# tgcsaba/GPSig

Measured on AMD Instinct MI355X. Metric: sequence-pairs/sec for SignatureKernel.K (N,L,d,sig_level); fp64 rel-err vs ref, higher is better.
Workload: dtype f64; 1 GPU; BASELINE.json configs[1]: full N x N Gram, SignatureLinear, N=4096, L=64, d=8, num_levels=5, order=1, normalization=on, fp64, white-noise inputs

## Files before the change

### gpsig_amd/csrc/api.hip

```cpp
#include <hip/hip_runtime.h>

#include <cstdarg>
#include <cstdio>
#include <cstdlib>
#include <cstring>
#include <string>
#include <vector>

#include "../../include/gpsig_hip.h"
#include "aux_kernels.hpp"
#include "lowrank_kernels.hpp"
#include "lr_fused_args.hpp"
#include "lr_draw_kernels.hpp"
#include "seq_args.hpp"
#include "seq_configs.hpp"
#include "tvs_tile_kernel.hpp"
#include "seq_pk2_kernel.hpp"
#include "sig_feat_kernel.hpp"

namespace gpsig {
typedef hipError_t (*TvsTileLaunchFn)(TvsTileArgs&, size_t, hipStream_t, int);
TvsTileLaunchFn tvs_tile_lookup(int M, int NW, int D, bool incr, int kind);
TvsTileLaunchFn tvs_tile_lookup_ho(int M, int NW, int D, bool incr);
int tvs_tile_width(int d);
// ... 633 lines not shown
    if (x_squared && (X2 == nullptr || raw || !p->normalization)) return GPSIG_OK;
    if (f32 && (row_end > 0 || row_block_call)) return GPSIG_OK;
    if (c->shard_n > 1) return GPSIG_OK;
    const int M = p->num_levels;
    if (M < 2 || p->order < 1 || p->order > M) return GPSIG_OK;
    const int d = p->num_features * ((raw ? 0 : p->num_lags) + 1);
    SigFeatLaunchFn ffn = sig_feat_lookup(d, M);
    if (!ffn) return GPSIG_OK;
    const bool sym = X2 == nullptr;
    void* out32 = nullptr;
    const void* const X_given = X;
    const int64_t F = sig_feature_count(d, M), ld = (F + 1 + 15) / 16 * 16;
    const int r1 = p->difference ? L1 - 1 : L1, r2 = p->difference ? L2 - 1 : L2;
    if (r1 < 1 || r2 < 1) return GPSIG_OK;
    if (c->sig_features < 0 && d != 1) {
        const double lattice = double(r1) * r2 * (2.0 * d + 3.0 * M - 1.0) * (p->order > 1 ? 8.0 : 1.0) * (cosine ? 1.5 : 1.0) * (f32 ? 0.5 : 1.0), feat = 2.0 * double(F);
        const double pairs = sym ? double(N1) * N1 / 2 : double(N1) * N2;
        if (!(feat * 0.6 < lattice)) return GPSIG_OK;
        const double seqs = double(N1) + (sym ? 0.0 : double(N2)), t_seq = 60e-6 * double(sig_ipow(d, M)) / 32768.0;
        const double t_feat_kernel = ceil(seqs / 256.0) * t_seq > 15e-6 ? ceil(seqs / 256.0) * t_seq : 15e-6;
        const double t_lattice = 100e-6 + pairs * lattice / (d > 8 ? 12.5e12 : 25e12), t_features = 60e-6 + t_feat_kernel + pairs * feat / 60e12;
        if (pairs < 1024.0 || !(t_features < t_lattice)) return GPSIG_OK;
    }
    const size_t lds = sig_features_lds_bytes(d, M, L1 > L2 ? L1 : L2);
    if (lds > 150 * 1024) return GPSIG_OK;
    const bool rows = row_end > 0 || row_block_call;
    const int64_t NA = rows ? row_end - row_begin : N1, H = N1 / 2;
    int64_t NB = sym ? N1 : N2;
    if (rows) NB = (NA + H < N1) ? NA + H : N1;
    const int nti = int((NA + SG_BM - 1) / SG_BM), ntj = int((NB + SG_BN - 1) / SG_BN);
    const bool symtiles = sym && !rows;
    const int ntiles = symtiles ? nti * (nti + 1) / 2 : nti * ntj;
    const int nslab_all = int((ld + SG_BK - 1) / SG_BK);
    int nsplit = 1, graded = 1;
    {
        const int64_t nt_full = (N1 + SG_BM - 1) / SG_BM;
        const int64_t tiles_full = sym ? nt_full * (nt_full + 1) / 2 : nt_full * ((N2 + SG_BN - 1) / SG_BN);
        const double result_bytes = 8.0 * double(N1) * double(sym ? N1 : N2) * (sym ? 0.5 : 1.0);
        double best = 1e300;
        for (int ns = 1; ns <= 128 && ns * 8 <= nslab_all + 7; ++ns) {
            const double wgs = double(tiles_full) * ns, per_piece = double(nslab_all) / ns;
            const double t = (wgs <= 256.0 ? per_piece * 1.8e-6 + 10e-6 : ceil(wgs / 512.0) * (per_piece * 3.6e-6 + 10e-6)) +
                             (ns > 1 ? 2.0 * ns * result_bytes / 3e12 : 0.0);
            if (t < best * 0.999) { best = t; nsplit = ns; }
        }
        if (tiles_full > 1024 && nsplit < 4 && nslab_all >= 32) nsplit = 4;
        const double wgs = double(tiles_full) * nsplit, piece_t = double(nslab_all) / nsplit * 3.6e-6;
        if (c->sig_graded != 0 && wgs > 512.0 && nslab_all / nsplit >= 32) {
            const double rounds = wgs / 512.0, waste_equal = (ceil(rounds) - rounds) * piece_t;
            double best_t = waste_equal;
            for (int g = 2; g <= 5; ++g) {
                const double t = piece_t / double(1 << (g - 1)) + (g - 1) * 2.0 * result_bytes / 3e12;
                if (t < best_t * 0.95 && (nslab_all / nsplit) >> (g - 1) >= 8) { best_t = t; graded = g; }
            }
        }
    }
    const size_t part_one = sizeof(double) * size_t(NA) * NB;
    while (nsplit > 1 && part_one * size_t(nsplit - 1 + graded) > (size_t(40) << 30)) { --nsplit; graded = 1; }
    const int npieces = nsplit - 1 + graded;
    const size_t feat_bytes = sizeof(double) * size_t(ld) * (size_t(N1) + (sym ? 0 : size_t(N2)));
    if (feat_bytes + part_one * size_t(npieces) > (size_t(96) << 30)) return GPSIG_OK;
    {
        auto grow = [&](int id, size_t bytes) { return bytes > c->buf[id].cap ? bytes + bytes / 8 + 256 : size_t(0); };
        const size_t extra = grow(B_SF0, sizeof(double) * size_t(ld) * N1 + 64) + (sym ? 0 : grow(B_SF1, sizeof(double) * size_t(ld) * N2 + 64)) +
                             grow(B_SF2, part_one * size_t(npieces) + 64);
        if (extra > (size_t(1) << 30) && !c->capturing && !rows) {
            size_t free_b = 0, total_b = 0;
            if (hipMemGetInfo(&free_b, &total_b) == hipSuccess) {
                size_t held = 0;
                for (int id : {int(B_SF0), int(B_SF1), int(B_SF2)}) held += grow(id, id == B_SF0 ? sizeof(double) * size_t(ld) * N1 + 64 : id == B_SF1 ? (sym ? 0 : sizeof(double) * size_t(ld) * N2 + 64) : part_one * size_t(npieces) + 64) ? c->buf[id].cap : 0;
                if (extra > free_b + held - (free_b + held) / 16) return GPSIG_OK;
            }
        }
    }
    if (rows && NA <= 0) { *done = true; return GPSIG_OK; }
    const double* w = nullptr;
    if (!raw) CHK(upload_weights(c, p, &w));
    ScaleParams s;
    CHK(scale_params(c, p, !raw, &s));
    void *phi1, *phi2 = nullptr, *part;
    CHK(ensure(c, B_SF0, sizeof(double) * size_t(ld) * N1 + 64, &phi1));
    if (!sym) CHK(ensure(c, B_SF1, sizeof(double) * size_t(ld) * N2 + 64, &phi2));
    CHK(ensure(c, B_SF2, part_one * size_t(npieces) + 64, &part));
    if (f32) {
        void *x64, *y64 = nullptr, *o64;
        const int64_t per1 = int64_t(L1) * p->num_features, per2 = int64_t(L2) * p->num_features;
        CHK(ensure(c, B_SF3, sizeof(double) * size_t(N1 * per1) + 64, &x64));
        HIPCHK(c, sig_convert_launch(X, x64, N1 * per1, true, c->stream));
        if (!sym) {
            CHK(ensure(c, B_SF4, sizeof(double) * size_t(N2 * per2) + 64, &y64));
            HIPCHK(c, sig_convert_launch(X2, y64, N2 * per2, true, c->stream));
        }
        CHK(ensure(c, B_SF5, sizeof(double) * size_t(return_levels ? M + 1 : 1) * size_t(N1) * size_t(sym ? N1 : N2) + 64, &o64));
        out32 = out; X = x64; X2 = sym ? nullptr : y64; out = o64;
    }
    const int normalize = (!raw && p->normalization) ? 1 : 0;
    auto features = [&](const void* Xs, int64_t N, int L, void* phi, bool squared) -> int {
        SigFeatArgs A;
        memset(&A, 0, sizeof(A));
        A.X = static_cast<const double*>(Xs); A.N = N; A.L = L; A.difference = p->difference ? 1 : 0; A.P = s;
        A.w = w; A.normalize = normalize; A.jitter = p->jitter; A.Phi = static_cast<double*>(phi); A.ld = ld; A.dlev = nullptr;
        A.order = p->order;
        A.unit_points = cosine ? 1 : 0;
        A.norm_squared = squared ? 1 : 0;
        const int64_t cap = sig_threads(d, M) <= 128 ? 16384 : 4096;
        const unsigned grid = unsigned(N < cap ? N : cap);
        hipError_t e = ffn(A, grid, sig_features_lds_bytes(d, M, L), c->stream);
        if (e != hipSuccess) return fail(c, GPSIG_ERR_HIP, "sig_features_kernel: %s", hipGetErrorString(e));
        return GPSIG_OK;
    };
    uint64_t key = 1469598103934665603ull;
    auto mix = [&](const void* ptr, size_t bytes) {
        const unsigned char* b = static_cast<const unsigned char*>(ptr);
        for (size_t i = 0; i < bytes; ++i) { key ^= b[i]; key *= 1099511628211ull; }
    };
    {
        const int32_t head[8] = {p->base_kernel, p->dtype, p->num_features, p->num_levels, p->order, p->difference, p->normalization, p->num_lags};
        mix(head, sizeof(head));
        mix(&p->sigma, sizeof(double)); mix(&p->jitter, sizeof(double));
        mix(p->variances, sizeof(double) * (M + 1));
        if (p->lengthscales) mix(p->lengthscales, sizeof(double) * p->num_features);
        if (p->num_lags > 0) { mix(p->lags, sizeof(double) * p->num_lags); mix(p->gamma, sizeof(double) * (p->num_lags + 1)); }
        const int64_t tail[4] = {N1, L1, (raw ? 1 : 0) + (x_squared ? 2 : 0), ld};
        mix(tail, sizeof(tail));
    }
    const bool reuse = c->sf_keep && c->sf_valid && c->sf_X == X_given && c->sf_phi == phi1 && c->sf_key == key;
    if (N1 > 0 && !reuse) CHK(features(X, N1, L1, phi1, x_squared != 0));
    c->sf_valid = c->sf_keep != 0 && N1 > 0;
    c->sf_X = X_given; c->sf_phi = phi1; c->sf_key = key;
    if (!sym && N2 > 0) CHK(features(X2, N2, L2, phi2, false));
    if (NA <= 0 || NB <= 0) { *done = true; return GPSIG_OK; }
    const int nlev = return_levels ? M + 1 : 1;
    const int64_t Ncols = sym ? N1 : N2;
    for (int lv = 0; lv < nlev; ++lv) {
        int kb = 0, ke = int(F) + 1;
        double dval = 0.0;
        if (return_levels) {
            if (lv == 0) { kb = int(F); ke = int(F) + 1; }
            else { kb = sig_feature_count(d, lv - 1); ke = sig_feature_count(d, lv); }
            dval = raw ? 0.0 : p->sigma * p->variances[lv];
        } else {
            for (int m = 0; m <= M; ++m) dval += p->sigma * p->variances[m];
        }
        SigGramArgs G;
        memset(&G, 0, sizeof(G));
        G.A = static_cast<const double*>(phi1) + (rows ? row_begin * ld : 0);
        G.B = static_cast<const double*>(sym ? phi1 : phi2);
        G.NA = NA; G.NB = NB; G.lda = ld; G.ldb = ld;
        G.b_off = rows ? ((row_begin - H) % N1 + N1) % N1 : 0; G.b_mod = sym ? N1 : N2;
        G.k_begin = kb; G.k_end = ke;
        G.band = (rows && NA + H <= N1) ? H : 0;
        const int nslab = (ke - kb + SG_BK - 1) / SG_BK;
        const int ns = sig_piece_bounds(nslab, nsplit, return_levels ? 1 : graded, G.bound);
        G.nsplit = ns; G.symmetric = symtiles ? 1 : 0; G.ntj = ntj; G.part = static_cast<double*>(part);
        hipEvent_t e0 = nullptr, e1 = nullptr;
        bool on = false;
        if (timed) CHK(timing_begin_any(c, &e0, &e1, &on));
        int used_dma = 0;
        HIPCHK(c, sig_gram_launch(G, ntiles, c->stream, (c->sig_gemm_dma && !return_levels) ? 1 : 0, &used_dma));
        if (on) {
            HIPCHK(c, hipEventRecord(e1, c->stream));
            c->t_launches += 1;
            c->t_pairs += NA * NB;
            c->t_kernel = used_dma ? "sig_gram_dma_kernel" : "sig_gram_kernel";
            c->t_flops += 2.0 * double(ntiles) * SG_BM * SG_BN * double(nslab) * SG_BK;
        }
        SigReduceArgs R;
        memset(&R, 0, sizeof(R));
        R.part = static_cast<const double*>(part); R.nsplit = ns; R.NA = NA; R.NB = NB;
        R.out = static_cast<double*>(out) + (return_levels ? int64_t(lv) * N1 * Ncols : 0);
        R.so_i = Ncols; R.so_j = 1;
        R.mode = rows ? 2 : (symtiles ? 1 : 0);
        R.diag_set = (sym && normalize) ? 1 : 0; R.diag_value = dval;
        R.N = N1; R.r0 = row_begin; R.c0 = G.b_off; R.compact = compact;
        HIPCHK(c, sig_reduce_launch(R, c->stream));
    }
    if (out32) HIPCHK(c, sig_convert_launch(out, out32, int64_t(return_levels ? M + 1 : 1) * N1 * (sym ? N1 : N2), false, c->stream));
    *done = true;
    return GPSIG_OK;
}

template <typename TT>
struct Impl {
struct SeqPlanned {
    SeqConfig cfg;
    SeqLaunchFn fn;
    int mode, d_eff;
    bool rbf_prescaled;
    int fast_kind;
    double prescale;
    bool pk2;
    int ny, waves;
};

static int plan_seq(gpsig_ctx* c, const gpsig_params* p, int d_eff, int Ly, SeqPlanned* out, int64_t pairs_hint = 0) {
    SeqGeom g0 = seq_geometry(p->base_kernel, p->difference, Ly, 4, int(sizeof(TT)));
    out->rbf_prescaled = false;
    out->fast_kind = -1;
    out->prescale = 1.0;
    out->pk2 = false;
    out->ny = 1; out->waves = 1;
    if (p->base_kernel == GPSIG_BASE_SPECTRAL) {
        int k = -1;
        if (sizeof(TT) == 8 && c->spectral_wave != 0 && g0.mode == MODE_PT_DIFF && !(p->order > 1 && p->num_levels > 1))
            k = seq_select(SEQ_TABLE_SPECTRAL, N_SEQ_TABLE_SPECTRAL, g0.rows, d_eff, p->num_levels, false);
        if (k < 0) return fail(c, GPSIG_ERR_UNSUPPORTED, "the spectral base kernel: no wavefront kernel for this shape / dtype / order");
        out->cfg = SEQ_TABLE_SPECTRAL[k];
        out->mode = g0.mode;
        out->d_eff = d_eff;
        out->fn = out->cfg.G == 16 ? seq_lookup_ptd_spectral_g16(out->cfg.G, out->cfg.C, out->cfg.D, out->cfg.MMAX, false)
                                   : seq_lookup_ptd_spectral_g64(out->cfg.G, out->cfg.C, out->cfg.D, out->cfg.MMAX, false);
        if (!out->fn) return fail(c, GPSIG_ERR_UNSUPPORTED, "spectral seq-gram kernel shape missing from this build");
        return GPSIG_OK;
    }
    if (p->order > 1 && p->num_levels > 1) {
        int k = seq_select_ho(SEQ_HO_TABLE, N_SEQ_HO_TABLE, g0.rows, d_eff, p->num_levels, p->order);
        if (k < 0)
            return fail(c, GPSIG_ERR_UNSUPPORTED,
                        "no higher-order seq-gram kernel shape for %d record rows, d=%d, num_levels=%d, order=%d (built: order <= 8 up "
                        "to 64 rows, <= 4 up to 128 rows, 2 up to 512 rows; num_levels <= 6 (8 up to 64 rows); d <= 16, or d <= 32 with at most 128 rows)",
                        g0.rows, d_eff, p->num_levels, p->order);
        const SeqHOConfig& h = SEQ_HO_TABLE[k];
        out->cfg = SeqConfig{h.G, h.C, h.D, h.MMAX, false};
        out->mode = g0.mode;
        out->d_eff = d_eff;
        out->fn = seq_launcher_ho(g0.mode, h, sizeof(TT) == 4);
        if (sizeof(TT) == 8 && c->allow_exact && g0.mode == MODE_PT_DIFF && p->base_kernel == GPSIG_BASE_RBF) {
            SeqLaunchFn ex = seq_lookup_ho_ptdrbf_exact(h.G, h.C, h.D, p->num_levels, p->order);
            if (!ex) ex = seq_lookup_ho_ptdrbf_exact_o4(h.G, h.C, h.D, p->num_levels, p->order);
            if (ex) {
                out->fn = ex;
                out->cfg = SeqConfig{h.G, h.C, h.D, p->num_levels, true};
                out->rbf_prescaled = true;
                out->prescale = SEQ_RBF_PRESCALE;
            }
        }
        if (sizeof(TT) == 8 && c->allow_exact && g0.mode == MODE_PT_DIFF && seq_is_matern(p->base_kernel) && c->matern_fast != 0) {
            SeqLaunchFn ex = p->base_kernel == GPSIG_BASE_MATERN12 ? seq_lookup_ho_ptdm12_exact(BASE_MATERN12, h.G, h.C, h.D, p->num_levels, p->order)
                             : (p->base_kernel == GPSIG_BASE_MATERN32 ? seq_lookup_ho_ptdm32_exact(BASE_MATERN32, h.G, h.C, h.D, p->num_levels, p->order)
                                                                      : seq_lookup_ho_ptdm52_exact(BASE_MATERN52, h.G, h.C, h.D, p->num_levels, p->order));
            if (ex) {
                out->fn = ex;
                out->cfg = SeqConfig{h.G, h.C, h.D, p->num_levels, true};
                out->rbf_prescaled = true;
                out->prescale = seq_matern_prescale(p->base_kernel);
            }
        }
        if (!out->fn) return fail(c, GPSIG_ERR_UNSUPPORTED, "higher-order kernel shape missing from this build");
        return GPSIG_OK;
    }
    const bool f32 = sizeof(TT) == 4;
    if (f32 && c->allow_pk2 && c->allow_exact && (g0.mode == MODE_INC || (g0.mode == MODE_PT_DIFF && p->base_kernel == GPSIG_BASE_RBF))) {
        int G, C, D;
// ... 1103 lines not shown
    if (e != hipSuccess) return fail(nullptr, GPSIG_ERR_HIP, "hipSetDevice(%d): %s", device, hipGetErrorString(e));
    hipDeviceProp_t prop;
    e = hipGetDeviceProperties(&prop, device);
    if (e != hipSuccess) return fail(nullptr, GPSIG_ERR_HIP, "hipGetDeviceProperties: %s", hipGetErrorString(e));
    if (strncmp(prop.gcnArchName, "gfx950", 6) != 0)
        return fail(nullptr, GPSIG_ERR_UNSUPPORTED, "device %d is %s; this library carries gfx950 (MI355X) code only", device, prop.gcnArchName);
    gpsig_ctx* c = new gpsig_ctx();
    c->device = device;
    c->num_cus = prop.multiProcessorCount;
    c->stream = static_cast<hipStream_t>(stream);
    const char* g = getenv("GPSIG_GLDS");
    c->use_glds = g ? atoi(g) : 1;
    const char* ex = getenv("GPSIG_NO_EXACT");
    c->allow_exact = (ex && atoi(ex)) ? 0 : 1;
    *out = c;
    return GPSIG_OK;
}

void gpsig_ctx_destroy(gpsig_ctx* c) {
    if (!c) return;
    (void)hipSetDevice(c->device);
    (void)hipStreamSynchronize(c->stream);
    for (DevBuf& b : c->buf)
        if (b.p) (void)hipFree(b.p);
    for (TaskSlot& t : c->task_slots)
        if (t.buf.p) (void)hipFree(t.buf.p);
    for (hipEvent_t e : c->ev) (void)hipEventDestroy(e);
    if (c->probe_stream) { if (c->probe_stop) *c->probe_stop = 1; (void)hipStreamSynchronize(c->probe_stream); (void)hipStreamDestroy(c->probe_stream); }
    if (c->probe_buf) (void)hipFree(c->probe_buf);
    if (c->side_stream) { (void)hipStreamSynchronize(c->side_stream); (void)hipStreamDestroy(c->side_stream); }
    if (c->side_fork) (void)hipEventDestroy(c->side_fork);
    if (c->side_join) (void)hipEventDestroy(c->side_join);
    for (int k = 0; k < 2; ++k) {
        if (c->pin[k]) (void)hipHostFree(c->pin[k]);
        if (c->pin_ev[k]) (void)hipEventDestroy(c->pin_ev[k]);
    }
    if (c->probe_stop) (void)hipHostFree(const_cast<int*>(c->probe_stop));
    solver_release(c->blas_handle);
    for (gpsig_lr_state* st : c->lr_states) { st->device = c->device; st->ctx = nullptr; }
    delete c;
}

const char* gpsig_last_error(gpsig_ctx* c) { return c ? c->err.c_str() : g_create_error.c_str(); }

int gpsig_set_pointer_mode(gpsig_ctx* c, int mode) {
    if (!c) return GPSIG_ERR_INVALID;
    if (mode != GPSIG_PTR_HOST && mode != GPSIG_PTR_DEVICE) return fail(c, GPSIG_ERR_INVALID, "unknown pointer mode %d", mode);
    c->ptr_mode = mode;
    return GPSIG_OK;
}

int gpsig_sync(gpsig_ctx* c) {
    if (!c) return GPSIG_ERR_INVALID;
    CHK(host_sync(c));
    return GPSIG_OK;
}

int gpsig_set_shard(gpsig_ctx* c, int index, int count) {
    if (!c) return GPSIG_ERR_INVALID;
    if (count < 1 || index < 0 || index >= count) return fail(c, GPSIG_ERR_INVALID, "bad shard (%d of %d)", index, count);
    c->shard_i = index;
    c->shard_n = count;
    return GPSIG_OK;
}

int gpsig_set_option(gpsig_ctx* c, const char* name, int value) {
    if (!c || !name) return GPSIG_ERR_INVALID;
    if (!strcmp(name, "glds")) c->use_glds = value ? 1 : 0;
    else if (!strcmp(name, "exact")) c->allow_exact = value ? 1 : 0;
    else if (!strcmp(name, "max_run")) c->max_run = value > 0 ? value : 0;
    else if (!strcmp(name, "tensor_lanes")) c->tens_lanes = value;
    else if (!strcmp(name, "grad_scratch_mb")) c->grad_scratch_mb = value > 0 ? value : 4096;
    else if (!strcmp(name, "grad_impl")) c->grad_impl = value;
    else if (!strcmp(name, "grad_stash_mb")) c->grad_stash_mb = value;
    else if (!strcmp(name, "matern_fast")) c->matern_fast = value;
    else if (!strcmp(name, "grad_fused_piece")) c->grad_fused_piece = value;
    else if (!strcmp(name, "tvs_zreg")) c->tvs_zreg = value;
    else if (!strcmp(name, "tvs_grad_tile")) c->tvs_grad_tile = value;
    else if (!strcmp(name, "pinned_staging")) c->pinned_staging = value ? 1 : 0;
    else if (!strcmp(name, "lr_jacobi")) c->lr_jacobi = value ? 1 : 0;
    else if (!strcmp(name, "sig_features")) c->sig_features = value;
    else if (!strcmp(name, "sig_gemm_dma")) c->sig_gemm_dma = value;
    else if (!strcmp(name, "sig_graded")) c->sig_graded = value;
    else if (!strcmp(name, "lr_grad_threads")) c->lr_grad_threads = value;
    else if (!strcmp(name, "sig_features_grad")) c->sig_features_grad = value;
    else if (!strcmp(name, "sig_features_keep")) { c->sf_keep = value; c->sf_valid = false; }
    else if (!strcmp(name, "keep_reset")) c->keep_reset = value ? 1 : 0;
    else if (!strcmp(name, "pk2")) c->allow_pk2 = value;
    else if (!strcmp(name, "f32_pack")) c->f32_pack = value;
    else if (!strcmp(name, "f32_waves")) c->f32_waves = value;
    else if (!strcmp(name, "tvs_tile")) c->tvs_tile = value;
    else if (!strcmp(name, "wide")) c->wide = value;
    else if (!strcmp(name, "wide_chunk_mb")) c->wide_chunk_mb = value > 0 ? value : 0;
    else if (!strcmp(name, "wide_contract")) c->wide_contract = value;
    else if (!strcmp(name, "wide_lat_waves")) c->wide_lat_waves = value;
    else if (!strcmp(name, "wide_sym_fold")) c->wide_sym_fold = value ? 1 : 0;
    else if (!strcmp(name, "ho_g32")) c->ho_g32 = value;
    else if (!strcmp(name, "wide_few_cols")) c->wide_few_cols = value;
    else if (!strcmp(name, "tvs_grad_matern")) c->tvs_grad_matern = value ? 1 : 0;
    else if (!strcmp(name, "wide_o1_sweeps")) c->wide_o1_sweeps = value;
    else if (!strcmp(name, "tvs_features")) c->tvs_features = value;
    else if (!strcmp(name, "tvs_tile_nw")) c->tvs_tile_nw = value;
    else if (!strcmp(name, "diag_own")) c->diag_own = value;
    else if (!strcmp(name, "spectral_wave")) c->spectral_wave = value;
    else if (!strcmp(name, "tens_tile")) c->tens_tile = value;
    else if (!strcmp(name, "lr_gemm")) c->lr_gemm = value;
    else if (!strcmp(name, "lr_fused")) c->lr_fused = value;
    else if (!strcmp(name, "lr_fused_variant")) c->lr_fused_variant = value;
    else if (!strcmp(name, "lr_fused_pad")) c->lr_fused_pad = value >= 0 ? value : 1;
    else return fail(c, GPSIG_ERR_INVALID, "unknown option '%s'", name);
    return GPSIG_OK;
}

int gpsig_graph_begin(gpsig_ctx* c) {
    if (!c) return GPSIG_ERR_INVALID;
    if (c->capturing) return fail(c, GPSIG_ERR_INVALID, "a graph capture is already open on this context");
    if (c->ptr_mode != GPSIG_PTR_DEVICE) return fail(c, GPSIG_ERR_INVALID, "graph capture needs device-pointer mode (gpsig_set_pointer_mode)");
    if (c->stream == nullptr) return fail(c, GPSIG_ERR_INVALID, "the default stream cannot be captured: create the context on a stream of its own");
    HIPCHK(c, hipSetDevice(c->device));
    HIPCHK(c, hipStreamBeginCapture(c->stream, hipStreamCaptureModeRelaxed));
    c->capturing = true;
    c->capture_failed = false;
    return GPSIG_OK;
}

int gpsig_graph_end(gpsig_ctx* c, gpsig_graph** out) {
    if (!c || !out) return GPSIG_ERR_INVALID;
    *out = nullptr;
    if (!c->capturing) return fail(c, GPSIG_ERR_INVALID, "no graph capture is open on this context");
    c->capturing = false;
    hipGraph_t g = nullptr;
    const hipError_t e = hipStreamEndCapture(c->stream, &g);
    if (c->capture_failed) {
        if (g) (void)hipGraphDestroy(g);
        (void)hipGetLastError();
        return GPSIG_ERR_INVALID;
    }
    if (e != hipSuccess || !g) return fail(c, GPSIG_ERR_HIP, "hipStreamEndCapture failed: %s", hipGetErrorString(e));
    gpsig_graph* G = new (std::nothrow) gpsig_graph();
    if (!G) { (void)hipGraphDestroy(g); return fail(c, GPSIG_ERR_NOMEM, "out of host memory"); }
    G->graph = g; G->ctx = c; G->alloc_gen = c->alloc_gen;
    const hipError_t ei = hipGraphInstantiate(&G->exec, g, nullptr, nullptr, 0);
    if (ei != hipSuccess) {
        (void)hipGraphDestroy(g);
        delete G;
        return fail(c, GPSIG_ERR_HIP, "hipGraphInstantiate failed: %s", hipGetErrorString(ei));
    }
    *out = G;
    return GPSIG_OK;
}

int gpsig_graph_launch(gpsig_ctx* c, gpsig_graph* G) {
    if (!c || !G) return GPSIG_ERR_INVALID;
    if (G->ctx != c) return fail(c, GPSIG_ERR_INVALID, "the graph was recorded on another context");
    if (c->capturing) return fail(c, GPSIG_ERR_INVALID, "a graph capture is open on this context");
    if (G->alloc_gen != c->alloc_gen)
        return fail(c, GPSIG_ERR_INVALID, "scratch buffers moved since the graph was recorded (a later call needed more memory, other task lists or other level weights): record it again");
    HIPCHK(c, hipSetDevice(c->device));
    HIPCHK(c, hipGraphLaunch(G->exec, c->stream));
    return GPSIG_OK;
}

void gpsig_graph_destroy(gpsig_graph* G) {
    if (!G) return;
    if (G->exec) (void)hipGraphExecDestroy(G->exec);
    if (G->graph) (void)hipGraphDestroy(G->graph);
// ... 812 lines not shown
```

### gpsig_amd/csrc/ctx.hpp

```cpp
#pragma once
#include <atomic>

#include <hip/hip_runtime.h>

#include <cstdarg>
#include <cstdio>
#include <cstdlib>
#include <cstring>
#include <string>
#include <thread>
#include <vector>

#include "../../include/gpsig_hip.h"
#include "seq_args.hpp"

struct DevBuf {
    void* p = nullptr;
    size_t cap = 0;
};

enum BufId {
    B_IN0, B_IN1, B_IN2,
    B_OUT0, B_OUT1, B_OUT2,
    B_REC0, B_REC1,
    B_DLEV0, B_DLEV1,
    B_FAC0, B_FAC1,
    B_TASKS, B_W, B_XT, B_ZT, B_ZS, B_ZL, B_ZN, B_TMP0, B_TMP1,
    B_LS, B_LR0, B_LR1, B_LR2, B_LR3, B_LR4, B_LR5, B_LR6, B_LR7, B_LR8,
    B_GR0, B_GR1, B_GR2, B_GR3, B_GR4, B_GR5, B_GR6, B_GR7,
    B_GR7B, B_TW0, B_TW1, B_TW2,
    B_SF0, B_SF1, B_SF2, B_SF3, B_SF4, B_SF5,
    B_SPEC,
    B_TQ,
    B_STASH,
    B_WD0, B_WD1, B_WD2, B_WD3, B_WD4, B_WD5, B_WD6, B_WD7, B_WD8, B_WD9, B_WD10,
    B_COUNT
};

inline thread_local std::string g_create_error;

struct TaskCache {
    int64_t key[10] = {0};
    int ntasks = 0;
    bool valid = false;
    bool match(const int64_t (&k)[10]) const {
        if (!valid) return false;
        for (int i = 0; i < 10; ++i) if (key[i] != k[i]) return false;
        return true;
    }
    void set(const int64_t (&k)[10], int n) { for (int i = 0; i < 10; ++i) key[i] = k[i]; ntasks = n; valid = true; }
};

struct TaskSlot {
    TaskCache tc;
    DevBuf buf;
    uint64_t stamp = 0;
    int64_t aux = 0;
};
constexpr size_t TASK_SLOTS = 16;

inline int64_t next_stash_generation() {
    static std::atomic<int64_t> counter{0};
    return ++counter;
}

struct gpsig_ctx {
    int device = 0;
    int num_cus = 256;
    hipStream_t stream = nullptr;
    int ptr_mode = GPSIG_PTR_HOST;
    int shard_i = 0, shard_n = 1;
    int use_glds = 1;
    int allow_exact = 1;
    int keep_reset = 1;
    int f32_pack = 2, f32_waves = 0;
    int allow_pk2 = 1;
    int max_run = 0;
    int tens_lanes = -1;
    int grad_scratch_mb = 4096;
    int matern_fast = 1;
    int grad_fused_piece = 0;
    int grad_stash_mb = 4096;
    bool stash_want = false;
    int64_t stash_desc[8] = {0, 0, 0, 0, 0, 0, 0, 0};
    int64_t stash_gen = 0;
    int grad_impl = 0;
    void* blas_handle = nullptr;
    int tvs_tile = -1;
    int wide = -1;
    int wide_contract = 1, wide_lat_waves = -1, wide_sym_fold = 1, ho_g32 = -1, wide_few_cols = 0, tvs_grad_matern = 1, wide_o1_sweeps = 1;
    int wide_chunk_mb = 0;
    int tvs_features = -1;
    int tvs_tile_nw = 0;
    int tens_tile = 1;
    int spectral_wave = 1;
    int diag_own = 1;
    int lr_gemm = 1;
    int lr_fused_pad = 1;
    int lr_fused_variant = 0;
    int lr_fused = 1;
    double* tvs_aux_out = nullptr;
    bool tvs_aux_written = false;
    int tvs_grad_tile = 1;
    int sig_features = -1;
    int sf_keep = 0;
    bool sf_valid = false;
    const void* sf_X = nullptr; const void* sf_phi = nullptr; uint64_t sf_key = 0;
    int sig_features_grad = -1;
    int lr_grad_threads = 1024;
    int sig_graded = 1;
    int sig_gemm_dma = 1;
    int lr_jacobi = 1;
    int tvs_zreg = -1;
    std::string err;
    DevBuf buf[B_COUNT];
    std::vector<gpsig::SeqTask> host_tasks;
    std::vector<TaskSlot> task_slots;
    uint64_t task_clock = 0;
    std::vector<double> last_weights;
    std::vector<double> last_ls;
    void* ls_base = nullptr;
    std::vector<double> last_spec;
    void* spec_base = nullptr;
    uint64_t lr_hash = 0;
    void* lr_base = nullptr;
    std::vector<size_t> lr_offsets;
    int64_t lr_off_key[3] = {-1, -1, -1};
    void* lr_off_base = nullptr;
    uint64_t lrg_hash = 0;
    void* lrg_base = nullptr;
    std::vector<size_t> lrg_offsets;
    std::vector<hipEvent_t> ev;
    size_t ev_used = 0;
    int64_t t_launches = 0, t_pairs = 0;
    const char* t_kernel = nullptr;
    double t_flops = 0.0;
    bool capturing = false, capture_failed = false;
    uint64_t alloc_gen = 0;
    hipStream_t probe_stream = nullptr;
    unsigned long long* probe_buf = nullptr;
    int probe_cap = 0, probe_n = 0;
    static constexpr int PROBE_WAVES = 8;
    double probe_ghz[PROBE_WAVES] = {};
    int probe_xcc[PROBE_WAVES] = {};
    int probe_waves = 0;
    void* pin[2] = {nullptr, nullptr};
    size_t pin_bytes = 0;
    hipEvent_t pin_ev[2] = {nullptr, nullptr};
    int pinned_staging = 1;
    hipStream_t side_stream = nullptr;
    hipEvent_t side_fork = nullptr, side_join = nullptr;
    volatile int* probe_stop = nullptr;
    std::vector<struct gpsig_lr_state*> lr_states;
};

struct gpsig_graph {
    hipGraph_t graph = nullptr;
    hipGraphExec_t exec = nullptr;
    uint64_t alloc_gen = 0;
    gpsig_ctx* ctx = nullptr;
};

inline int fail(gpsig_ctx* c, int code, const char* fmt, ...) {
    char tmp[512];
    va_list ap;
    va_start(ap, fmt);
    vsnprintf(tmp, sizeof(tmp), fmt, ap);
    va_end(ap);
    if (c) c->err = tmp; else g_create_error = tmp;
    return code;
}

#define HIPCHK(c, expr)                                                                                         \
    do {                                                                                                        \
        hipError_t e__ = (expr);                                                                                \
        if (e__ != hipSuccess) return fail((c), GPSIG_ERR_HIP, "%s failed: %s", #expr, hipGetErrorString(e__)); \
    } while (0)
#define CHK(expr)                    \
    do {                             \
        int rc__ = (expr);           \
        if (rc__ != GPSIG_OK) return rc__; \
    } while (0)

inline int no_capture(gpsig_ctx* c, const char* what) {
    if (!c->capturing) return GPSIG_OK;
    c->capture_failed = true;
    return fail(c, GPSIG_ERR_INVALID, "graph capture: %s -- run the same calls once before gpsig_graph_begin", what);
}

#ifdef __HIPCC__
#ifdef GPSIG_KERNEL_DEFS
__global__ void zero_fill_kernel(unsigned long long* p, size_t n8, unsigned char* tail, int ntail) {
    const size_t stride = size_t(gridDim.x) * blockDim.x;
    for (size_t i = size_t(blockIdx.x) * blockDim.x + threadIdx.x; i < n8; i += stride) p[i] = 0ull;
// ... 218 lines not shown
```

### gpsig_amd/csrc/sig_feat_kernel.hpp

```cpp
#pragma once

#include <hip/hip_runtime.h>
#include <stdint.h>

#include <type_traits>

#include "aux_kernels.hpp"
#include "sig_pieces.hpp"

namespace gpsig {

constexpr int sig_ipow(int d, int m) {
    long long v = 1;
    for (int i = 0; i < m; ++i) { v *= d; if (v > (1ll << 30)) return 1 << 30; }
    return int(v);
}
constexpr int sig_lower_total(int d, int M) { int s = 0; for (int m = 1; m < M; ++m) s += sig_ipow(d, m); return s; }
constexpr int sig_feature_count(int d, int M) { int s = 0; for (int m = 1; m <= M; ++m) s += sig_ipow(d, m); return s; }
constexpr int SIG_MAX_TOP = 32768;
constexpr int sig_threads(int d, int M) {
    int t = 64;
    while (t < 512 && t * 64 < sig_ipow(d, M)) t *= 2;
    return t;
}
// ... 318 lines not shown
            __syncthreads();
            if (tid >= 1 && tid <= M) {
                double t = 0.0;
                for (int k2 = 0; k2 < NW; ++k2) t += red[k2 * (M + 1) + tid];
                norms[tid] = t;
            }
            __syncthreads();
        }
        double* out = A.Phi + n * A.ld;
        auto scale_of = [&](int m) {
            const double w = A.w ? A.w[m] : 1.0;
            const double nm = m == 0 ? 1.0 : norms[m];
            return A.normalize ? (A.norm_squared ? sqrt(w) / (nm + A.jitter) : sqrt(w / (nm + A.jitter))) : sqrt(w);
        };
        int off = 0;
#pragma unroll
        for (int m = 1; m <= M - 2; ++m) {
            const int k = M - 1 - m;
            if (own[k]) out[off + tid / sig_ipow(D, k - 1)] = scale_of(m) * anc[k];
            off += sig_ipow(D, m);
        }
        {
            const double sc = scale_of(M - 1);
#pragma unroll
            for (int q = 0; q < D; ++q) out[off + q * T + tid] = sc * par[q];
            off += sig_ipow(D, M - 1);
        }
        {
            const double sc = scale_of(M);
            if constexpr (D % 2 == 0) {
                double2* o2 = reinterpret_cast<double2*>(out + off);
#pragma unroll
                for (int q = 0; q < D; ++q)
#pragma unroll
                    for (int f = 0; f < D; f += 2) o2[(q * (D / 2) + f / 2) * T + tid] = double2{sc * top[q][f], sc * top[q][f + 1]};
            } else {
#pragma unroll
                for (int q = 0; q < D; ++q)
#pragma unroll
                    for (int f = 0; f < D; ++f) out[off + (q * D + f) * T + tid] = sc * top[q][f];
            }
            off += sig_ipow(D, M);
        }
        for (int64_t e = off + tid; e < A.ld; e += T) out[e] = e == off ? scale_of(0) : 0.0;
        if (A.dlev && tid <= M) A.dlev[n * (M + 1) + tid] = tid == 0 ? 1.0 : norms[tid];
    }
}

inline size_t sig_features_lds_bytes(int d, int M, int L) {
    (void)M;
    return sizeof(double) * ((size_t(L) + (d <= 64 ? 64 / d : 1)) * d + 64 + 64 + size_t(L) * d + size_t(L));
}

#ifdef GPSIG_KERNEL_DEFS
__global__ void sig_widen_kernel(const float* __restrict__ in, double* __restrict__ out, int64_t n) {
    for (int64_t i = blockIdx.x * int64_t(blockDim.x) + threadIdx.x; i < n; i += int64_t(gridDim.x) * blockDim.x) out[i] = double(in[i]);
}
#else
__global__ void sig_widen_kernel(const float* __restrict__ in, double* __restrict__ out, int64_t n);
#endif
#ifdef GPSIG_KERNEL_DEFS
__global__ void sig_narrow_kernel(const double* __restrict__ in, float* __restrict__ out, int64_t n) {
    for (int64_t i = blockIdx.x * int64_t(blockDim.x) + threadIdx.x; i < n; i += int64_t(gridDim.x) * blockDim.x) out[i] = float(in[i]);
}
#else
__global__ void sig_narrow_kernel(const double* __restrict__ in, float* __restrict__ out, int64_t n);
#endif

typedef double sig_f64x4 __attribute__((ext_vector_type(4)));
constexpr int SG_BM = 128, SG_BN = 128, SG_BK = 16, SG_LDK = SG_BK + 1;
constexpr int SG_MAX_PIECES = 144;

struct SigGramArgs {
    const double* A; const double* B;
    int64_t NA, NB, lda, ldb;
    int64_t b_off, b_mod;
    int k_begin, k_end;
    int nsplit;
    int bound[SG_MAX_PIECES + 1];
    int symmetric;
    int ntj;
    double* part;
    int64_t band;
};

__device__ inline void sig_tile_of(const SigGramArgs& G, int& split_out, int& bi, int& bj) {
    const int ntiles = gridDim.x / G.nsplit;
    const int split = blockIdx.x / ntiles;
    int tile;
    {
        const int j = blockIdx.x - split * ntiles, off = (split * ntiles) & 7, x = (off + j) & 7;
        int start = 0;
        for (int xp = 0; xp < x; ++xp) {
            const int j0 = (xp - off + 8) & 7;
            start += j0 < ntiles ? (ntiles - 1 - j0) / 8 + 1 : 0;
        }
        tile = start + ((j - ((x - off + 8) & 7)) >> 3);
    }
    {
        constexpr int SB = 8;
        const int nti = G.symmetric ? G.ntj : (ntiles / G.ntj), nbi = (nti + SB - 1) / SB, nbj = (G.ntj + SB - 1) / SB;
        int Bi = 0, Bj = 0, hi = 0, wj = 0;
        bool found = false;
        for (Bi = 0; Bi < nbi && !found; ++Bi) {
            hi = nti - Bi * SB < SB ? nti - Bi * SB : SB;
            for (Bj = G.symmetric ? Bi : 0; Bj < nbj; ++Bj) {
                wj = G.ntj - Bj * SB < SB ? G.ntj - Bj * SB : SB;
                const int cnt = (G.symmetric && Bj == Bi) ? hi * (hi + 1) / 2 : hi * wj;
                if (tile < cnt) { found = true; break; }
                tile -= cnt;
            }
            if (found) break;
        }
        int li_, lj_;
        if (G.symmetric && Bj == Bi) {
            li_ = 0;
            int rowlen = hi;
            while (tile >= rowlen) { tile -= rowlen; ++li_; --rowlen; }
            lj_ = li_ + tile;
        } else {
            li_ = tile / wj;
            lj_ = tile - li_ * wj;
        }
        bi = Bi * SB + li_;
        bj = Bj * SB + lj_;
    }
    split_out = split;
}

template <bool VEC>
static __global__ __launch_bounds__(256, 2) void sig_gram_kernel(const SigGramArgs G) {
    __shared__ double As[2][SG_BM * SG_LDK];
    __shared__ double Bs[2][SG_BN * SG_LDK];
    const int tid = threadIdx.x, wave = tid >> 6, lane = tid & 63;
    const int wr = wave >> 1, wc = wave & 1;
    const int li = lane & 15, lk = lane >> 4;
    int split, bi, bj;
    sig_tile_of(G, split, bi, bj);
    const int64_t tile_i = int64_t(bi) * SG_BM, tile_j = int64_t(bj) * SG_BN;
    if (G.band > 0 && (tile_j + SG_BN - 1 < tile_i || tile_j > tile_i + SG_BM - 1 + G.band)) return;
    const int s0 = G.bound[split], s1 = G.bound[split + 1];
    const int kb = G.k_begin + s0 * SG_BK, ke = (G.k_begin + s1 * SG_BK < G.k_end) ? G.k_begin + s1 * SG_BK : G.k_end;
    const int srow = tid >> 1, scol = (tid & 1) * 8;
    const int64_t ai = tile_i + srow, bjr = tile_j + srow;
    const bool aok = ai < G.NA, bok = bjr < G.NB;
    int64_t brow_i = G.b_off + (bok ? bjr : 0);
    if (brow_i >= G.b_mod) brow_i -= G.b_mod;
    const double* arow = G.A + (aok ? ai : 0) * G.lda;
    const double* brow = G.B + brow_i * G.ldb;
    double pa[8], pb[8];
    auto fetch = [&](int k0) {
        if (VEC && k0 + SG_BK <= ke) {
            const double2* a2 = reinterpret_cast<const double2*>(arow + k0 + scol);
            const double2* b2 = reinterpret_cast<const double2*>(brow + k0 + scol);
#pragma unroll
            for (int e = 0; e < 4; ++e) {
                const double2 va = a2[e], vb = b2[e];
                pa[2 * e] = va.x; pa[2 * e + 1] = va.y;
                pb[2 * e] = vb.x; pb[2 * e + 1] = vb.y;
            }
        } else {
#pragma unroll
            for (int e = 0; e < 8; ++e) {
                const int k = k0 + scol + e;
                pa[e] = (aok && k < ke) ? arow[k] : 0.0;
                pb[e] = (bok && k < ke) ? brow[k] : 0.0;
// ... 74 lines not shown
        int64_t brow_i = G.b_off + (bjr < G.NB ? bjr : 0);
        if (brow_i >= G.b_mod) brow_i -= G.b_mod;
        ga[q] = G.A + (ai < G.NA ? ai : 0) * G.lda + G.k_begin + int64_t(s0) * SG_BK + 2 * p;
        gb[q] = G.B + brow_i * G.ldb + G.k_begin + int64_t(s0) * SG_BK + 2 * p;
    }
    auto dma = [&](auto buf_c, auto ahead_c) {
        constexpr int BUF = decltype(buf_c)::value, OFF = decltype(ahead_c)::value * SG_BK * 8;
#pragma unroll
        for (int q = 0; q < 4; ++q) {
            __builtin_amdgcn_global_load_lds((const __attribute__((address_space(1))) void*)ga[q],
                                             (__attribute__((address_space(3))) void*)(&As[BUF][(q * 4 + wave) * 8 * SG_BK] - OFF / 8), 16, OFF, 0);
            __builtin_amdgcn_global_load_lds((const __attribute__((address_space(1))) void*)gb[q],
                                             (__attribute__((address_space(3))) void*)(&Bs[BUF][(q * 4 + wave) * 8 * SG_BK] - OFF / 8), 16, OFF, 0);
        }
    };
    auto advance = [&](int slabs) {
#pragma unroll
        for (int q = 0; q < 4; ++q) { ga[q] += slabs * SG_BK; gb[q] += slabs * SG_BK; }
    };
    const int swz = (lk >> 1) ^ ((li >> 1) & 7);
    int fo[4];
#pragma unroll
    for (int kq = 0; kq < 4; ++kq) fo[kq] = (((2 * kq) ^ swz) << 1) + (lk & 1) + li * SG_BK;
    const double* const Aw = &As[0][wr * 64 * SG_BK];
    const double* const Bw = &Bs[0][wc * 64 * SG_BK];
    auto frag = [&](auto buf_c, int kq, double (&av)[4], double (&bv)[4]) {
        constexpr int BUF = decltype(buf_c)::value;
#pragma unroll
        for (int m = 0; m < 4; ++m) {
            av[m] = Aw[BUF * SG_BM * SG_BK + m * 16 * SG_BK + fo[kq]];
            bv[m] = Bw[BUF * SG_BN * SG_BK + m * 16 * SG_BK + fo[kq]];
        }
    };
    sig_f64x4 acc[4][4];
#pragma unroll
    for (int m = 0; m < 4; ++m)
#pragma unroll
        for (int n = 0; n < 4; ++n) acc[m][n] = sig_f64x4{0.0, 0.0, 0.0, 0.0};
    double fa[2][4], fb[2][4];
    using B0 = std::integral_constant<int, 0>;
    using B1 = std::integral_constant<int, 1>;
    if (nsl > 0) dma(B0{}, B0{});
    asm volatile("s_waitcnt vmcnt(0)" ::: "memory");
    __syncthreads();
    if (nsl > 0) frag(B0{}, 0, fa[0], fb[0]);
    auto slab = [&](auto buf_c, auto ahead_c, bool more) {
        constexpr int BUF = decltype(buf_c)::value;
        using OTHER = std::integral_constant<int, BUF ^ 1>;
        if (more) dma(OTHER{}, ahead_c);
#pragma unroll
        for (int kq = 0; kq < 4; ++kq) {
            const int cur = kq & 1, nxt = cur ^ 1;
            if (kq < 3) {
                frag(buf_c, kq + 1, fa[nxt], fb[nxt]);
            } else {
                asm volatile("s_waitcnt vmcnt(0)" ::: "memory");
                __syncthreads();
                if (more) frag(OTHER{}, 0, fa[nxt], fb[nxt]);
            }
#pragma unroll
            for (int m = 0; m < 4; ++m)
#pragma unroll
                for (int n = 0; n < 4; ++n) acc[m][n] = __builtin_amdgcn_mfma_f64_16x16x4f64(fa[cur][m], fb[cur][n], acc[m][n], 0, 0, 0);
        }
    };
    int s = 0;
    for (; s + 8 <= nsl; s += 8) {
        slab(B0{}, std::integral_constant<int, 1>{}, true);
        slab(B1{}, std::integral_constant<int, 2>{}, true);
        slab(B0{}, std::integral_constant<int, 3>{}, true);
        slab(B1{}, std::integral_constant<int, 4>{}, true);
        slab(B0{}, std::integral_constant<int, 5>{}, true);
        slab(B1{}, std::integral_constant<int, 6>{}, true);
        slab(B0{}, std::integral_constant<int, 7>{}, true);
        slab(B1{}, std::integral_constant<int, 8>{}, s + 8 < nsl);
        advance(8);
    }
    for (; s + 2 <= nsl; s += 2) {
        slab(B0{}, std::integral_constant<int, 1>{}, true);
        slab(B1{}, std::integral_constant<int, 2>{}, s + 2 < nsl);
        advance(2);
    }
    if (s < nsl) slab(B0{}, std::integral_constant<int, 1>{}, false);
    double* const P = G.part + int64_t(split) * G.NA * G.NB;
#pragma unroll
    for (int m = 0; m < 4; ++m)
#pragma unroll
        for (int n = 0; n < 4; ++n)
#pragma unroll
            for (int r = 0; r < 4; ++r) {
                const int64_t i = tile_i + wr * 64 + m * 16 + lk + 4 * r, j = tile_j + wc * 64 + n * 16 + li;
                if (i < G.NA && j < G.NB) P[i * G.NB + j] = acc[m][n][r];
            }
}
#else
__global__ __launch_bounds__(256, 2) void sig_gram_dma_kernel(const SigGramArgs G);
#endif

struct SigReduceArgs {
    const double* part; int nsplit; int64_t NA, NB;
    double* out; int64_t so_i, so_j;
    int mode, diag_set; double diag_value;
    int64_t N, r0, c0;
    int compact;
};
#ifdef GPSIG_KERNEL_DEFS
__global__ void sig_gram_reduce_sym_kernel(const SigReduceArgs R, int nt) {
    __shared__ double tile[32][33];
    int t = blockIdx.y, bi = 0, rowlen = nt;
    while (t >= rowlen) { t -= rowlen; ++bi; --rowlen; }
    const int bj = bi + t;
    constexpr int SB = SG_BM / 32;
    const int sbi = blockIdx.x / SB, sbj = blockIdx.x - sbi * SB;
    const int64_t i0 = int64_t(bi) * SG_BM + sbi * 32, j0 = int64_t(bj) * SG_BN + sbj * 32;
    const int64_t stride = R.NA * R.NB;
    for (int r = threadIdx.y; r < 32; r += 8) {
        const int64_t i = i0 + r, j = j0 + threadIdx.x;
        double s = 0.0;
        if (i < R.NA && j < R.NB) {
            for (int k = 0; k < R.nsplit; ++k) s += R.part[int64_t(k) * stride + i * R.NB + j];
            if (i == j && R.diag_set) s = R.diag_value;
            R.out[i * R.so_i + j * R.so_j] = s;
        }
        tile[r][threadIdx.x] = s;
    }
    if (bi == bj) return;
    __syncthreads();
    for (int r = threadIdx.y; r < 32; r += 8) {
        const int64_t j = j0 + r, i = i0 + threadIdx.x;
        if (i < R.NA && j < R.NB) R.out[j * R.so_i + i * R.so_j] = tile[threadIdx.x][r];
    }
}
#else
__global__ void sig_gram_reduce_sym_kernel(const SigReduceArgs R, int nt);
#endif

#ifdef GPSIG_KERNEL_DEFS
__global__ void sig_gram_reduce_kernel(const SigReduceArgs R) {
    const int64_t total = R.NA * R.NB, stride = R.NA * R.NB;
    for (int64_t e = blockIdx.x * int64_t(blockDim.x) + threadIdx.x; e < total; e += int64_t(gridDim.x) * blockDim.x) {
        const int64_t i = e / R.NB, j = e - i * R.NB;
        int64_t src = e;
        if (R.mode == 1 && (i / SG_BM) > (j / SG_BN)) src = j * R.NB + i;
        double s = 0.0;
        if (R.mode == 2) {
            const int64_t seq_j = R.r0 + i;
            int64_t seq_i = R.c0 + j;
            if (seq_i >= R.N) seq_i -= R.N;
            const int64_t H = R.N / 2;
            int64_t dlt = seq_j - seq_i;
            if (dlt < 0) dlt += R.N;
            const bool own = dlt < H || (dlt == H && ((R.N & 1) || seq_i < seq_j));
            if (!own) continue;
            for (int k = 0; k < R.nsplit; ++k) s += R.part[int64_t(k) * stride + src];
            if (dlt == 0 && R.diag_set) s = R.diag_value;
            if (R.compact) R.out[i * (H + 1) + H - dlt] = s;
            else R.out[i * R.N + seq_i] = s;
            continue;
        }
        for (int k = 0; k < R.nsplit; ++k) s += R.part[int64_t(k) * stride + src];
        if (R.mode == 1 && i == j && R.diag_set) s = R.diag_value;
        R.out[i * R.so_i + j * R.so_j] = s;
    }
}
#else
__global__ void sig_gram_reduce_kernel(const SigReduceArgs R);
#endif

}
```

Baseline: 1.759 billion sequence-pairs/s.

## Fuse split-K reduction into Gram DMA kernel via last-arriving-block counter

```diff
diff --git a/gpsig_amd/csrc/api.hip b/gpsig_amd/csrc/api.hip
--- a/gpsig_amd/csrc/api.hip
+++ b/gpsig_amd/csrc/api.hip
@@ -739,6 +739,14 @@
     CHK(ensure(c, B_SF0, sizeof(double) * size_t(ld) * N1 + 64, &phi1));
     if (!sym) CHK(ensure(c, B_SF1, sizeof(double) * size_t(ld) * N2 + 64, &phi2));
     CHK(ensure(c, B_SF2, part_one * size_t(npieces) + 64, &part));
+    unsigned* tile_count = nullptr;
+    if (symtiles && !return_levels && c->sig_fuse_reduce && c->sig_gemm_dma) {
+        const size_t had = c->buf[B_SFC].cap;
+        void* cnt;
+        CHK(ensure(c, B_SFC, sizeof(unsigned) * size_t(nti) * size_t(ntj) + 64, &cnt));
+        if (c->buf[B_SFC].cap != had) CHK(zero_async(c, cnt, c->buf[B_SFC].cap));
+        tile_count = static_cast<unsigned*>(cnt);
+    }
     if (f32) {
         void *x64, *y64 = nullptr, *o64;
         const int64_t per1 = int64_t(L1) * p->num_features, per2 = int64_t(L2) * p->num_features;
@@ -810,6 +818,9 @@
         const int nslab = (ke - kb + SG_BK - 1) / SG_BK;
         const int ns = sig_piece_bounds(nslab, nsplit, return_levels ? 1 : graded, G.bound);
         G.nsplit = ns; G.symmetric = symtiles ? 1 : 0; G.ntj = ntj; G.part = static_cast<double*>(part);
+        double* const out_lv = static_cast<double*>(out) + (return_levels ? int64_t(lv) * N1 * Ncols : 0);
+        G.count = tile_count; G.out = out_lv; G.ldo = Ncols;
+        G.diag_set = (sym && normalize) ? 1 : 0; G.diag_value = dval;
         hipEvent_t e0 = nullptr, e1 = nullptr;
         bool on = false;
         if (timed) CHK(timing_begin_any(c, &e0, &e1, &on));
@@ -822,10 +833,11 @@
             c->t_kernel = used_dma ? "sig_gram_dma_kernel" : "sig_gram_kernel";
             c->t_flops += 2.0 * double(ntiles) * SG_BM * SG_BN * double(nslab) * SG_BK;
         }
+        if (tile_count && used_dma) continue;
         SigReduceArgs R;
         memset(&R, 0, sizeof(R));
         R.part = static_cast<const double*>(part); R.nsplit = ns; R.NA = NA; R.NB = NB;
-        R.out = static_cast<double*>(out) + (return_levels ? int64_t(lv) * N1 * Ncols : 0);
+        R.out = out_lv;
         R.so_i = Ncols; R.so_j = 1;
         R.mode = rows ? 2 : (symtiles ? 1 : 0);
         R.diag_set = (sym && normalize) ? 1 : 0; R.diag_value = dval;
@@ -2095,6 +2107,7 @@
     else if (!strcmp(name, "sig_features")) c->sig_features = value;
     else if (!strcmp(name, "sig_gemm_dma")) c->sig_gemm_dma = value;
     else if (!strcmp(name, "sig_graded")) c->sig_graded = value;
+    else if (!strcmp(name, "sig_fuse_reduce")) c->sig_fuse_reduce = value;
     else if (!strcmp(name, "lr_grad_threads")) c->lr_grad_threads = value;
     else if (!strcmp(name, "sig_features_grad")) c->sig_features_grad = value;
     else if (!strcmp(name, "sig_features_keep")) { c->sf_keep = value; c->sf_valid = false; }
diff --git a/gpsig_amd/csrc/ctx.hpp b/gpsig_amd/csrc/ctx.hpp
--- a/gpsig_amd/csrc/ctx.hpp
+++ b/gpsig_amd/csrc/ctx.hpp
@@ -32,6 +32,7 @@
     B_SF0, B_SF1, B_SF2, B_SF3, B_SF4, B_SF5,
     B_SPEC,
     B_TQ,
+    B_SFC,
     B_STASH,
     B_WD0, B_WD1, B_WD2, B_WD3, B_WD4, B_WD5, B_WD6, B_WD7, B_WD8, B_WD9, B_WD10,
     B_COUNT
@@ -110,6 +111,7 @@
     int lr_grad_threads = 1024;
     int sig_graded = 1;
     int sig_gemm_dma = 1;
+    int sig_fuse_reduce = 1;
     int lr_jacobi = 1;
     int tvs_zreg = -1;
     std::string err;
diff --git a/gpsig_amd/csrc/sig_feat_kernel.hpp b/gpsig_amd/csrc/sig_feat_kernel.hpp
--- a/gpsig_amd/csrc/sig_feat_kernel.hpp
+++ b/gpsig_amd/csrc/sig_feat_kernel.hpp
@@ -424,6 +424,9 @@
     int ntj;
     double* part;
     int64_t band;
+    unsigned* count;
+    double* out; int64_t ldo;
+    int diag_set; double diag_value;
 };
 
 __device__ inline void sig_tile_of(const SigGramArgs& G, int& split_out, int& bi, int& bj) {
@@ -664,7 +667,8 @@
         advance(2);
     }
     if (s < nsl) slab(B0{}, std::integral_constant<int, 1>{}, false);
-    double* const P = G.part + int64_t(split) * G.NA * G.NB;
+    const int64_t stride = G.NA * G.NB;
+    double* const P = G.part + int64_t(split) * stride;
 #pragma unroll
     for (int m = 0; m < 4; ++m)
 #pragma unroll
@@ -674,6 +678,84 @@
                 const int64_t i = tile_i + wr * 64 + m * 16 + lk + 4 * r, j = tile_j + wc * 64 + n * 16 + li;
                 if (i < G.NA && j < G.NB) P[i * G.NB + j] = acc[m][n][r];
             }
+    if (!G.count) return;
+    int* const last_flag = reinterpret_cast<int*>(lds_all);
+    asm volatile("s_waitcnt vmcnt(0)" ::: "memory");
+    __syncthreads();
+    if (tid == 0) {
+        unsigned* const cnt = G.count + int64_t(bi) * G.ntj + bj;
+        __builtin_amdgcn_fence(__ATOMIC_RELEASE, "agent");
+        asm volatile("s_waitcnt vmcnt(0)" ::: "memory");
+        const unsigned arrived = __hip_atomic_fetch_add(cnt, 1u, __ATOMIC_RELAXED, __HIP_MEMORY_SCOPE_AGENT);
+        const int last = arrived == unsigned(G.nsplit - 1);
+        if (last) {
+            __builtin_amdgcn_fence(__ATOMIC_ACQUIRE, "agent");
+            __hip_atomic_store(cnt, 0u, __ATOMIC_RELAXED, __HIP_MEMORY_SCOPE_AGENT);
+            asm volatile("s_waitcnt vmcnt(0)" ::: "memory");
+        }
+        *last_flag = last;
+    }
+    __syncthreads();
+    if (!__builtin_amdgcn_readfirstlane(*last_flag)) return;
+    double (*const T)[SG_BN + 1] = reinterpret_cast<double (*)[SG_BN + 1]>(lds_all + SG_GUARD);
+    const bool mirror = bi != bj;
+    const int64_t rstep = 4 * G.NB;
+#pragma unroll 1
+    for (int m = 0; m < 4; ++m) {
+        const int64_t i0 = tile_i + wr * 64 + m * 16 + lk, j0 = tile_j + wc * 64 + li;
+        double sum[4][4];
+#pragma unroll
+        for (int n = 0; n < 4; ++n)
+#pragma unroll
+            for (int r = 0; r < 4; ++r) sum[n][r] = 0.0;
+        auto piece = [&](int k, double (&v)[4][4]) {
+            const double* const Pk = G.part + int64_t(k) * stride + i0 * G.NB + j0;
+#pragma unroll
+            for (int r = 0; r < 4; ++r)
+#pragma unroll
+                for (int n = 0; n < 4; ++n) v[n][r] = (i0 + 4 * r < G.NA && j0 + 16 * n < G.NB) ? Pk[r * rstep + 16 * n] : 0.0;
+        };
+        int k = 0;
+        for (; k + 2 <= G.nsplit; k += 2) {
+            double v[2][4][4];
+            piece(k, v[0]);
+            piece(k + 1, v[1]);
+#pragma unroll
+            for (int n = 0; n < 4; ++n)
+#pragma unroll
+                for (int r = 0; r < 4; ++r) sum[n][r] = (sum[n][r] + v[0][n][r]) + v[1][n][r];
+        }
+        for (; k < G.nsplit; ++k) {
+            double v[4][4];
+            piece(k, v);
+#pragma unroll
+            for (int n = 0; n < 4; ++n)
+#pragma unroll
+                for (int r = 0; r < 4; ++r) sum[n][r] += v[n][r];
+        }
+        double* const O = G.out + i0 * G.ldo + j0;
+#pragma unroll
+        for (int r = 0; r < 4; ++r)
+#pragma unroll
+            for (int n = 0; n < 4; ++n) {
+                double v = sum[n][r];
+                if (i0 + 4 * r == j0 + 16 * n && G.diag_set) v = G.diag_value;
+                if (i0 + 4 * r < G.NA && j0 + 16 * n < G.NB) O[(4 * r) * G.ldo + 16 * n] = v;
+                if (mirror) T[wr * 16 + lk + 4 * r][wc * 64 + n * 16 + li] = v;
+            }
+        if (mirror) {
+            __syncthreads();
+            const int il = tid & 31;
+            const int64_t i = tile_i + (il >> 4) * 64 + m * 16 + (il & 15);
+#pragma unroll
+            for (int q = 0; q < SG_BN / 8; ++q) {
+                const int jl = (tid >> 5) + 8 * q;
+                const int64_t j = tile_j + jl;
+                if (i < G.NA && j < G.NB) G.out[j * G.ldo + i] = T[il][jl];
+            }
+            __syncthreads();
+        }
+    }
 }
 #else
 __global__ __launch_bounds__(256, 2) void sig_gram_dma_kernel(const SigGramArgs G);
```

Result: no change. 1.762 billion sequence-pairs/s (median of 6 runs) (+0.2%).
